# drprojects/DeepViewAgg

Hardware: AMD Instinct MI355X
Metric: points/sec fused fwd+bwd (1M pts, 32 views) (higher is better)
Workload: dtype bf16

## Files before the change

### deepviewagg_amd/_lib.py

```python
import ctypes
import os

_HERE = os.path.dirname(os.path.abspath(__file__))
LIB_PATH = os.environ.get("DVA_LIB_PATH") or os.path.join(_HERE, "csrc", "libdva_hip.so")

DVA_F32, DVA_BF16, DVA_F16 = 0, 1, 2
DVA_SUM, DVA_MEAN, DVA_MAX, DVA_MIN = 0, 1, 2, 3
REDUCE_CODE = {"sum": DVA_SUM, "add": DVA_SUM, "mean": DVA_MEAN, "max": DVA_MAX, "min": DVA_MIN}
CAMERA_CODE = {
    "s3dis_equirectangular": 0,
    "scannet": 1,
    "kitti360_perspective": 2,
    "kitti360_fisheye": 3,
}

_ERRORS = {
    -1: "DVA_ERR_INVALID (bad argument)",
    -2: "DVA_ERR_UNSUPPORTED",
    -3: "DVA_ERR_LAUNCH (HIP runtime error)",
    -4: "DVA_ERR_OVERFLOW (composite key does not fit int64)",
}


class DvaError(RuntimeError):
# ... 83 lines not shown
    "dva_rowbn_bwd_apply": (ctypes.c_int, [_vp, _vp, _vp, _vp, _vp, _vp, _i64, _i32, _f32, _i32, _vp]),
    "dva_bn_finalize": (ctypes.c_int, [_vp, ctypes.c_double, _vp, _vp, _vp, _vp, _vp, _f32, _f32, _i32, _i32, _vp,
                                       _vp]),
    "dva_scale_f64": (ctypes.c_int, [_vp, ctypes.c_double, _vp, _i32, _vp]),
    "dva_chain_prep": (ctypes.c_int, [_vp, _vp, _vp, _i32, _vp, _vp, _i32, _vp, _vp]),
    "dva_chain_tile_count": (ctypes.c_int, [_vp, _vp, _i32, _vp, _vp]),
    "dva_chain_tile_build": (ctypes.c_int, [_vp, _vp, _i32, _vp, _vp, _vp]),
    "dva_chain_moments": (ctypes.c_int, [_vp, _i64, _vp, _i32, _vp, _vp, _vp]),
    "dva_chain_stats2": (ctypes.c_int, [_vp, _vp, _vp, _vp, _vp, _vp, _vp, _vp, _vp, _vp, _i64, _vp]),
    "dva_chain_pooled": (ctypes.c_int, [_vp, _vp, _vp, _vp, _i64, _vp]),
    "dva_chain_stats": (ctypes.c_int, [_i32, _vp, _vp, _vp, _vp, _vp, _vp, _vp, _vp, _vp, _vp, _i64, _i64, _vp]),
    "dva_chain_stats_a2": (ctypes.c_int, [_i32, _vp, _vp, _vp, _vp, _vp, _vp, _vp, _vp, _vp, _vp, _i64, _i64, _vp, _vp]),
    "dva_chain_score_stats_a2": (ctypes.c_int, [_vp] * 12 + [_i32, _i64, _i64, _vp]),
    "dva_chain_bwd_layer6_a2": (ctypes.c_int, [_vp] * 13 + [_i32, _i64, _i64, _vp]),
    "dva_chain_attn_fwd": (ctypes.c_int, [_vp] * 18 + [_i64, _i64, _i64, _i32, _i32, _i32, _f32, _vp]),
    "dva_chain_attn_bwd": (ctypes.c_int, [_vp] * 14 + [_i64, _i64, _i64, _i32, _i32, _i32, _f32, _vp]),
    "dva_chain_attn_fwd_dt": (ctypes.c_int, [_vp] * 18 + [_i64, _i64, _i64, _i32, _i32, _i32, _f32, _i32, _vp]),
    "dva_chain_attn_bwd_dt": (ctypes.c_int, [_vp] * 14 + [_i64, _i64, _i64, _i32, _i32, _i32, _f32, _i32, _vp]),
    "dva_chain_attn_bwd_f32": (ctypes.c_int, [_vp] * 14 + [_i64, _i64, _i64, _i32, _i32, _i32, _f32, _vp]),
    "dva_gather_segment_max_fwd": (ctypes.c_int, [_vp] * 5 + [_i64, _i64, _i64, _i32, _i32, _vp]),
    "dva_gather_segment_max_bwd": (ctypes.c_int, [_vp] * 8 + [_i64, _i64, _i64, _i32, _i32, _vp]),
    "dva_chain_keys": (ctypes.c_int, [_vp] * 12 + [_i64, _i64, _vp]),
    "dva_chain_keys_compat": (ctypes.c_int, [_vp] * 14 + [_i32, _f32, _i64, _i64, _vp]),
    "dva_chain_attn_fwd_keys": (ctypes.c_int, [_vp] * 12 + [_f32] + [_vp] * 8 + [_i64, _i64, _i64, _i32, _i32, _i32, _f32, _vp]),
    "dva_qkv_dquery": (ctypes.c_int, [_vp, _i32, _vp, _vp, _vp, _i64, _i64, _i32, _f32, _vp]),
    "dva_chain_score_stats_keys": (ctypes.c_int, [_vp] * 15 + [_i32, _f32, _i64, _i64, _vp]),
    "dva_chain_bwd_layer6_keys": (ctypes.c_int, [_vp] * 16 + [_i32, _f32, _i64, _i64, _vp]),
    "dva_qkv_compat": (ctypes.c_int, [_vp] * 4 + [_i64, _i32, _f32, _vp]),
    "dva_qkv_compat_bwd": (ctypes.c_int, [_vp] * 7 + [_i64, _i64, _i32, _f32, _vp]),
    "dva_chain_attn_bwd_planrec": (ctypes.c_int, [_vp] * 15 + [_i64, _i64, _i64, _i32, _i32, _i32, _f32, _vp]),
    "dva_plan_inverse": (ctypes.c_int, [_vp, _vp, _i64, _vp]),
    "dva_plan_split_table_bytes": (ctypes.c_int64, [_i64, _i64]),
    "dva_plan_split_build": (ctypes.c_int, [_vp, _i64, _i64, _vp, _vp, _vp, _i64, _vp, _i64, _vp]),
    "dva_plan_split_sort_records": (ctypes.c_int, [_vp, _vp, _i64, _i64, _vp, _vp, _i64, _vp, _vp, _vp]),
    "dva_plan_split_sort_records32": (ctypes.c_int, [_vp, _vp, _i64, _i64, _vp, _i64, _vp, _vp]),
    "dva_plan_split_rows_grad": (ctypes.c_int, [_vp, _vp, _i64, _i64, _vp, _i64, _vp, _i32, _i32, _i32, _i32, _vp]),
    "dva_chain_score_stats": (ctypes.c_int, [_vp] * 14 + [_i32, _i64, _i64, _vp]),
    "dva_chain_bwd_layer": (ctypes.c_int, [_i32] + [_vp] * 22 + [_i32, _i64, _i64, _vp]),
    "dva_gather_bilinear_taps_anchor": (ctypes.c_int, [_vp, _vp, _i64, _i32, _i32, _i32, _vp, _vp, _vp, _vp]),
    "dva_bilinear_taps_cat": (ctypes.c_int, [_i32, _vp, _vp, _vp, _vp, _vp, _vp, _vp, _i64, _vp, _vp, _vp, _vp]),
    "dva_anchor_rows_sum": (ctypes.c_int, [_vp, _vp, _vp, _vp, _vp, _i64, _i64, _i32, _i32, _vp]),
    "dva_anchor_combine": (ctypes.c_int, [_vp, _vp, _i32, _i32, _i32, _i32, _vp]),
    "dva_anchor_fixup": (ctypes.c_int, [_vp, _vp, _vp, _vp, _vp, _i64, _i32, _i32, _i32, _i32, _i32, _vp]),
    "dva_anchor_rows_sum_bn": (ctypes.c_int, [_vp] * 10 + [_i64, _i64, _i32, _vp]),
    "dva_anchor_fixup_bn": (ctypes.c_int, [_vp] * 8 + [_i64, _i32, _i32, _i32, _i32, _vp]),
    "dva_emod_prep": (ctypes.c_int, [_vp, _i32, _vp, _vp]),
    "dva_emod_stats": (ctypes.c_int, [_i32] + [_vp] * 9 + [_i64, _i64, _i32, _vp]),
    "dva_emod_attn_fwd": (ctypes.c_int, [_vp] * 23 + [_i64, _i64, _i64, _i32, _i32, _i32, _f32, _vp]),
    "dva_emod_attn_bwd": (ctypes.c_int, [_vp] * 20 + [_i64, _i64, _i64, _i32, _i32, _i32, _f32, _vp]),
    "dva_emod_stats1_plan": (ctypes.c_int, [_vp] * 6 + [_i64, _i64, _i32, _vp]),
    "dva_emod_bwd": (ctypes.c_int, [_i32] + [_vp] * 16 + [_i64, _i64, _i64, _i32, _i32, _vp]),
    "dva_chain_score_l6_stats": (ctypes.c_int, [_vp] * 16 + [_i32, _i64, _i64, _vp]),
    "dva_chain_l6_consts": (ctypes.c_int, [_vp] * 7),
    "dva_chain_bwd_layer5_merged": (ctypes.c_int, [_vp] * 18 + [_i32, _i64, _i64, _vp]),
    "dva_chain_route_stats": (ctypes.c_int, [_vp, _vp, _vp, _vp, _vp, _vp, _i64, _vp]),
    "dva_copy_ceiling": (ctypes.c_int, [_vp, _vp, _i64, _vp]),
    "dva_zero_unseen_rows": (ctypes.c_int, [_vp, _vp, _i64, _i64, _vp]),
    "dva_chain_bn_consts": (ctypes.c_int, [_vp, ctypes.c_double, _vp, _vp, _vp, _vp, _vp, ctypes.c_float, ctypes.c_float,
                                           _i32, _vp, _i32, _i32, _vp, _vp, _vp]),
    "dva_concat_cast_fwd": (ctypes.c_int, [_vp, _vp, _vp, _i64, _i32, _i32, _i32, _vp]),
    "dva_concat_cast_bwd": (ctypes.c_int, [_vp, _vp, _vp, _i64, _i32, _i32, _i32, _vp]),
    "dva_mapping_row_index": (ctypes.c_int, [_vp, _vp, _vp, _i32, ctypes.c_double, _i64, _i64, _i32, _i32, _i32, _vp, _vp]),
    "dva_view_gather_rows_grad_rec16": (ctypes.c_int, [_vp, _vp, _vp, _vp, _vp, _i64, _i64, _i32, _i32, _i32, _vp]),
    "dva_view_gather_rows_grad_rec16_to": (ctypes.c_int, [_vp, _vp, _vp, _vp, _vp, _i32, _i64, _i64, _i32, _i32, _i32, _vp]),
    "dva_chain_tile_chunks": (ctypes.c_int, [_vp, _i64, _i64, _i32, _vp, _vp]),
    "dva_chain_tile_offsets": (ctypes.c_int, [_vp, _i32, _vp, _vp, _vp]),
# ... 122 lines not shown
```

### deepviewagg_amd/csrc/dva_common.h

```cpp
#pragma once
#include <hip/hip_runtime.h>
#include <stdint.h>

#include <cstdlib>

#include "../../include/dva.h"

#define DVA_WAVE 64

#define DVA_CHECK_LAUNCH()                           \
  do {                                               \
    hipError_t e__ = hipGetLastError();              \
    if (e__ != hipSuccess) return DVA_ERR_LAUNCH;    \
  } while (0)

namespace dva {

static inline int tune_int(const char* name, int dflt) {
  const char* v = getenv(name);
  return v && *v ? atoi(v) : dflt;
}

typedef uint16_t bf16_t;

// ... 57 lines not shown
};
template <>
struct Elt<bf16_t> {
  static __device__ __forceinline__ float ld(const bf16_t* p, int64_t i) { return bf2f(p[i]); }
  static __device__ __forceinline__ void st(bf16_t* p, int64_t i, float v) { p[i] = f2bf(v); }
};
template <>
struct Elt<f16_t> {
  static __device__ __forceinline__ float ld(const f16_t* p, int64_t i) { return (float)p[i]; }
  static __device__ __forceinline__ void st(f16_t* p, int64_t i, float v) { p[i] = (f16_t)v; }
};

__host__ __device__ __forceinline__ int group_of_channel(int c, int C, int G) {
  if (G <= 1) return 0;
  if (G >= C) return c;
  const int base = C / G, rem = C % G;
  const int split = rem * (base + 1);
  return c < split ? c / (base + 1) : rem + (c - split) / base;
}
__host__ __device__ __forceinline__ int group_begin(int g, int C, int G) {
  if (g >= G) return C;
  if (G <= 1) return 0;
  if (G >= C) return g;
  const int base = C / G, rem = C % G;
  return g < rem ? g * (base + 1) : rem * (base + 1) + (g - rem) * base;
}

struct __attribute__((aligned(8))) PackedIdx {
  int32_t img;
  int16_t x;
  int16_t y;
};

static inline int blocks_for(int64_t n, int threads) { return (int)((n + threads - 1) / threads); }

}
```

### deepviewagg_amd/csrc/gather.hip

```cpp
#include "dva_common.h"

namespace dva {

__device__ __forceinline__ float floordiv_f32(float a, float b) {
  const float mod = fmodf(a, b);
  float div = __fdiv_rn(__fsub_rn(a, mod), b);
  if (mod != 0.f && ((b < 0.f) != (mod < 0.f))) div = __fsub_rn(div, 1.f);
  if (div != 0.f) {
    float fl = floorf(div);
    if (__fsub_rn(div, fl) > 0.5f) fl = __fadd_rn(fl, 1.f);
    return fl;
  }
  return copysignf(0.f, __fdiv_rn(a, b));
}

template <typename PIX>
__global__ __launch_bounds__(256) void pack_index_kernel(const int64_t* __restrict__ images,
                                                          const int64_t* __restrict__ atom_ptr,
                                                          const PIX* __restrict__ pixels,
                                                          double ratio, int64_t n_views,
                                                          PackedIdx* __restrict__ out) {
  for (int64_t v = blockIdx.x * (int64_t)blockDim.x + threadIdx.x; v < n_views;
       v += (int64_t)gridDim.x * blockDim.x) {
    const int32_t img = (int32_t)images[v];
    for (int64_t a = atom_ptr[v]; a < atom_ptr[v + 1]; ++a) {
      PackedIdx pi;
      pi.img = img;
      if (ratio == 1.0) {
        pi.x = (int16_t)pixels[2 * a];
        pi.y = (int16_t)pixels[2 * a + 1];
      } else {
        const float rf = (float)ratio;
        pi.x = (int16_t)floordiv_f32((float)pixels[2 * a], rf);
        pi.y = (int16_t)floordiv_f32((float)pixels[2 * a + 1], rf);
      }
      out[a] = pi;
    }
  }
}

template <typename PIX>
__global__ __launch_bounds__(256) void mapping_row_index_kernel(const int64_t* __restrict__ images,
                                                                 const int64_t* __restrict__ atom_ptr,
                                                                 const PIX* __restrict__ pixels, double ratio,
                                                                 int64_t n_views, int H, int W,
                                                                 int32_t* __restrict__ row_idx) {
  for (int64_t v = blockIdx.x * (int64_t)blockDim.x + threadIdx.x; v < n_views;
       v += (int64_t)gridDim.x * blockDim.x) {
    const int32_t img = (int32_t)images[v];
    for (int64_t a = atom_ptr[v]; a < atom_ptr[v + 1]; ++a) {
      int32_t x, y;
      if (ratio == 1.0) {
        x = (int32_t)pixels[2 * a];
        y = (int32_t)pixels[2 * a + 1];
      } else {
        const float rf = (float)ratio;
        x = (int32_t)(int16_t)floordiv_f32((float)pixels[2 * a], rf);
        y = (int32_t)(int16_t)floordiv_f32((float)pixels[2 * a + 1], rf);
      }
      row_idx[a] = (img * H + y) * W + x;
    }
  }
}

__global__ __launch_bounds__(256) void row_index_kernel(const PackedIdx* __restrict__ idx,
                                                         int64_t n_atoms, int H, int W,
                                                         int32_t row_offset,
                                                         int32_t* __restrict__ row_idx,
                                                         int32_t* __restrict__ counts) {
  for (int64_t p = blockIdx.x * (int64_t)blockDim.x + threadIdx.x; p < n_atoms;
       p += (int64_t)gridDim.x * blockDim.x) {
    const PackedIdx pi = idx[p];
    const int32_t r = (pi.img * H + pi.y) * W + pi.x;
    row_idx[p] = r + row_offset;
    if (counts) atomicAdd(&counts[r], 1);
  }
}

template <typename UNIT>
__global__ __launch_bounds__(256) void gather_nearest_fwd_kernel(const UNIT* __restrict__ x,
                                                                  const PackedIdx* __restrict__ idx,
                                                                  UNIT* __restrict__ out,
                                                                  int64_t n_atoms, int H, int W,
                                                                  int units_per_row) {
  const int64_t total = n_atoms * (int64_t)units_per_row;
  for (int64_t t = blockIdx.x * (int64_t)blockDim.x + threadIdx.x; t < total;
       t += (int64_t)gridDim.x * blockDim.x) {
    const int64_t p = t / units_per_row;
    const int u = (int)(t - p * units_per_row);
    const PackedIdx pi = idx[p];
    const int64_t pix = ((int64_t)pi.img * H + pi.y) * W + pi.x;
    out[t] = x[pix * units_per_row + u];
  }
}
// ... 800 lines not shown
```

### deepviewagg_amd/csrc/plan_split.hip

```cpp
#include "dva_common.h"

namespace dva {
namespace ps {

constexpr int IPT = 8;
constexpr int BINS = 512;
constexpr int LO_BITS = 9;
constexpr int HEAD_INTS = 4096;

static inline int tile_size() {
  static const int t = tune_int("DVA_PLAN_TILE", 4096) == 8192 ? 8192 : 4096;
  return t;
}

struct Layout {
  int64_t nt, nb, ntb;
  size_t off_tot, off_bstart, off_tstart, off_order, off_a, off_b, off_desc, total;
};

static inline bool eligible(int64_t n_views, int64_t n_rows) {
  return n_views > 0 && n_views <= 0x7fffffffLL && n_rows > BINS && n_rows <= (int64_t)BINS * BINS;
}

static inline Layout layout(int64_t n, int64_t n_rows) {
  Layout L;
  const int TILE = tile_size();
  L.nt = (n + TILE - 1) / TILE;
  L.nb = (n_rows + BINS - 1) / BINS;
  L.ntb = L.nt + L.nb;
  L.off_tot = 0;
  L.off_bstart = 512 * 4;
  L.off_tstart = (512 + 520) * 4;
  L.off_order = 2048 * 4;
  L.off_a = HEAD_INTS * 4;
  L.off_b = L.off_a + (size_t)L.nt * BINS * 4;
  L.off_desc = L.off_b + (size_t)L.ntb * BINS * 4;
  L.total = L.off_desc + (size_t)L.ntb * 16;
  return L;
}

template <int NT>
// ... 28 lines not shown

template <int TILE>
__global__ __launch_bounds__(TILE / IPT) void hist_hi_kernel(const uint32_t* __restrict__ keys, int64_t n, int nb,
                                                             int64_t nt, int32_t* __restrict__ offA) {
  constexpr int THREADS = TILE / IPT;
  __shared__ int h[BINS];
  for (int i = threadIdx.x; i < BINS; i += THREADS) h[i] = 0;
  __syncthreads();
  const int64_t base = (int64_t)blockIdx.x * TILE;
#pragma unroll
  for (int k = 0; k < IPT; ++k) {
    const int64_t e = base + k * THREADS + threadIdx.x;
    if (e < n) atomicAdd(&h[hi_digit(keys[e], nb)], 1);
  }
  __syncthreads();
  for (int i = threadIdx.x; i < nb; i += THREADS) offA[(int64_t)i * nt + blockIdx.x] = h[i];
}

__global__ __launch_bounds__(256) void scan_tiles_kernel(int32_t* __restrict__ off, int64_t nt, int32_t* __restrict__ tot) {
  __shared__ int s_w[4];
  int32_t* row = off + (int64_t)blockIdx.x * nt;
  int carry = 0;
  for (int64_t t0 = 0; t0 < nt; t0 += 256) {
    const int64_t t = t0 + threadIdx.x;
    const int v = t < nt ? row[t] : 0;
    int all;
    const int ex = block_excl_scan<256>(v, s_w, &all);
    if (t < nt) row[t] = carry + ex;
    carry += all;
  }
  if (threadIdx.x == 0) tot[blockIdx.x] = carry;
}

__global__ __launch_bounds__(BINS) void bucket_starts_kernel(const int32_t* __restrict__ tot, int nb, int TILE,
                                                             int32_t* __restrict__ bucket_start,
                                                             int32_t* __restrict__ tile_start, int4* __restrict__ desc,
                                                             int32_t* __restrict__ order) {
  __shared__ int s_w[BINS / 64];
  __shared__ int s_tot[BINS];
  const int d = threadIdx.x;
  const int v = d < nb ? tot[d] : 0;
  s_tot[d] = d < nb ? v : -1;
  __syncthreads();
  if (d < nb) {
    int before = 0;
    for (int j = 0; j < nb; ++j) {
      const int t = s_tot[j];
      before += (t > v || (t == v && j < d)) ? 1 : 0;
    }
    order[before] = d;
  }
  int all;
  const int bs = block_excl_scan<BINS>(v, s_w, &all);
  bucket_start[d] = bs;
  if (d == BINS - 1) bucket_start[BINS] = all;
  int allt;
  const int nt_b = (v + TILE - 1) / TILE;
  const int ts = block_excl_scan<BINS>(nt_b, s_w, &allt);
  tile_start[d] = ts;
  if (d == BINS - 1) tile_start[BINS] = allt;
  for (int j = 0; j < nt_b; ++j) {
    const int left = v - j * TILE;
    desc[ts + j] = make_int4(d, bs + j * TILE, left < TILE ? left : TILE, 0);
  }
}

__device__ __forceinline__ void tile_b(const int4* __restrict__ desc, int tb, int& b, int64_t& start, int& count) {
  const int4 d = desc[tb];
  b = rfl_i(d.x);
  start = (int64_t)rfl_i(d.y);
  count = rfl_i(d.z);
}

template <int TILE>
__global__ __launch_bounds__(TILE / IPT) void hist_lo_kernel(const uint16_t* __restrict__ lows, int nb,
                                                             const int32_t* __restrict__ tile_start,
                                                             const int4* __restrict__ desc, int32_t* __restrict__ offB) {
  constexpr int THREADS = TILE / IPT;
  __shared__ int h[BINS];
  if ((int)blockIdx.x >= tile_start[nb]) return;
  int b, count;
  int64_t start;
  tile_b(desc, blockIdx.x, b, start, count);
  for (int i = threadIdx.x; i < BINS; i += THREADS) h[i] = 0;
  __syncthreads();
#pragma unroll
  for (int k = 0; k < IPT; ++k) {
    const int i = k * THREADS + threadIdx.x;
    if (i < count) atomicAdd(&h[lows[start + i]], 1);
  }
  __syncthreads();
  for (int i = threadIdx.x; i < BINS; i += THREADS) offB[(int64_t)blockIdx.x * BINS + i] = h[i];
}

__global__ __launch_bounds__(BINS) void scan_rows_kernel(int32_t* __restrict__ offB, const int32_t* __restrict__ bucket_start,
                                                         const int32_t* __restrict__ tile_start, int64_t n_rows,
                                                         int64_t n_views, int32_t* __restrict__ row_ptr,
// ... 361 lines not shown
          raw[u] = make_float4(0.f, 0.f, 0.f, 0.f);
          if (in) raw[u] = *reinterpret_cast<const float4*>(gout + p * C + cl * 4);
        }
#pragma unroll
        for (int u = 0; u < U; ++u) {
          acc[rr][0] = fmaf(raw[u].x, sc[u], acc[rr][0]);
          acc[rr][1] = fmaf(raw[u].y, sc[u], acc[rr][1]);
          acc[rr][2] = fmaf(raw[u].z, sc[u], acc[rr][2]);
          acc[rr][3] = fmaf(raw[u].w, sc[u], acc[rr][3]);
        }
      }
    }
  }
#pragma unroll
  for (int rr = 0; rr < RPT; ++rr) {
    const int64_t r = (int64_t)b * BINS + grp + GROUPS * rr;
    if (r < n_rows)
      *reinterpret_cast<float4*>(grows + r * C + cl * 4) = make_float4(acc[rr][0], acc[rr][1], acc[rr][2], acc[rr][3]);
  }
}

template <int C, typename T>
static void bucket_rows_grad(const uint4* rec, const T* gout, T* grows, int64_t n_rows, int G, int nb,
                             const int32_t* bstart, const int32_t* order, hipStream_t s) {
  static const int bt = tune_int("DVA_PLAN_BT", 8192);
  if (bt == 2048)
    hipLaunchKernelGGL((bucket_rows_grad_kernel<C, 2048, T>), dim3(nb), dim3(1024), 0, s, rec, gout, grows, n_rows, G, bstart, order);
  else if (bt == 4096)
    hipLaunchKernelGGL((bucket_rows_grad_kernel<C, 4096, T>), dim3(nb), dim3(1024), 0, s, rec, gout, grows, n_rows, G, bstart, order);
  else
    hipLaunchKernelGGL((bucket_rows_grad_kernel<C, 8192, T>), dim3(nb), dim3(1024), 0, s, rec, gout, grows, n_rows, G, bstart, order);
}

}
}

namespace dva {
namespace ps {
struct Tables {
  int32_t *tot, *bstart, *tstart, *order, *offA, *offB;
  int4* desc;
};
static inline Tables tables_of(void* tables, const Layout& L) {
  char* tb = (char*)tables;
  return {(int32_t*)(tb + L.off_tot), (int32_t*)(tb + L.off_bstart), (int32_t*)(tb + L.off_tstart),
          (int32_t*)(tb + L.off_order), (int32_t*)(tb + L.off_a), (int32_t*)(tb + L.off_b), (int4*)(tb + L.off_desc)};
}

static inline bool xcd_on() {
  static const int on = tune_int("DVA_PLAN_XCD", 1);
  return on != 0;
}
static inline unsigned scatter_grid(int64_t tiles) { return (unsigned)(xcd_on() ? (tiles + 7) / 8 * 8 : tiles); }

template <int TILE>
static void build(const uint32_t* keys, int64_t n, int64_t n_rows, int32_t* row_ptr, int32_t* counts, const Layout& L,
                  const Tables& T, void* scratch, hipStream_t s) {
  constexpr int THREADS = TILE / IPT;
  const int nb = (int)L.nb;
  hipLaunchKernelGGL(hist_hi_kernel<TILE>, dim3((unsigned)L.nt), dim3(THREADS), 0, s, keys, n, nb, L.nt, T.offA);
  hipLaunchKernelGGL(scan_tiles_kernel, dim3(nb), dim3(256), 0, s, T.offA, L.nt, T.tot);
  hipLaunchKernelGGL(bucket_starts_kernel, dim3(1), dim3(BINS), 0, s, T.tot, nb, TILE, T.bstart, T.tstart, T.desc, T.order);
  hipLaunchKernelGGL((scatter_kernel<MODE_LOWS, TILE>), dim3(scatter_grid(L.nt)), dim3(THREADS), 0, s, keys,
                     (const uint4*)nullptr, scratch, n, nb, n_rows, L.nt, T.bstart, T.tstart, T.desc, T.offA,
                     (const int32_t*)nullptr, (int)xcd_on());
  hipLaunchKernelGGL(hist_lo_kernel<TILE>, dim3((unsigned)L.ntb), dim3(THREADS), 0, s, (const uint16_t*)scratch, nb,
                     T.tstart, T.desc, T.offB);
  hipLaunchKernelGGL(scan_rows_kernel, dim3(nb), dim3(BINS), 0, s, T.offB, T.bstart, T.tstart, n_rows, n, row_ptr, counts);
}

template <int TILE>
static void sort_records(const uint32_t* keys, const uint4* rec, int64_t n, int64_t n_rows, const int32_t* row_ptr,
                         const Layout& L, const Tables& T, void* buf, void* out, hipStream_t s) {
  constexpr int THREADS = TILE / IPT;
  const int nb = (int)L.nb;
  hipLaunchKernelGGL((scatter_kernel<MODE_REC_A, TILE>), dim3(scatter_grid(L.nt)), dim3(THREADS), 0, s, keys, rec,
                     buf, n, nb, n_rows, L.nt, T.bstart, T.tstart, T.desc, T.offA, (const int32_t*)nullptr,
                     (int)xcd_on());
  if (!out) return;
  hipLaunchKernelGGL((scatter_kernel<MODE_REC_B, TILE>), dim3(scatter_grid(L.ntb)), dim3(THREADS), 0, s,
                     (const uint32_t*)nullptr, (const uint4*)buf, out, n, nb, n_rows, L.nt, T.bstart, T.tstart, T.desc,
                     T.offB, row_ptr, (int)xcd_on());
}
}
}

using namespace dva;

extern "C" {

int64_t dva_plan_split_table_bytes(int64_t n_views, int64_t n_rows) {
  if (n_views < 0 || n_rows < 0) return DVA_ERR_INVALID;
  if (!ps::eligible(n_views, n_rows)) return DVA_ERR_UNSUPPORTED;
  return (int64_t)ps::layout(n_views, n_rows).total;
}

int dva_plan_split_build(const int32_t* row_idx, int64_t n_views, int64_t n_rows, int32_t* row_ptr, int32_t* counts,
                         void* tables, int64_t tables_bytes, void* scratch, int64_t scratch_bytes, void* stream) {
  if (n_views < 0 || n_rows < 0) return DVA_ERR_INVALID;
  if (!ps::eligible(n_views, n_rows)) return DVA_ERR_UNSUPPORTED;
  if (!row_idx || !row_ptr || !tables || !scratch) return DVA_ERR_INVALID;
  const ps::Layout L = ps::layout(n_views, n_rows);
  if ((int64_t)L.total > tables_bytes || scratch_bytes < n_views * 2) return DVA_ERR_INVALID;
  const ps::Tables T = ps::tables_of(tables, L);
  if (ps::tile_size() == 4096)
    ps::build<4096>((const uint32_t*)row_idx, n_views, n_rows, row_ptr, counts, L, T, scratch, (hipStream_t)stream);
  else
    ps::build<8192>((const uint32_t*)row_idx, n_views, n_rows, row_ptr, counts, L, T, scratch, (hipStream_t)stream);
  DVA_CHECK_LAUNCH();
  return DVA_OK;
}

int dva_plan_split_sort_records(const int32_t* row_idx, const void* rec, int64_t n_views, int64_t n_rows,
                                const int32_t* row_ptr, const void* tables, int64_t tables_bytes, void* buf,
                                void* rec_sorted, void* stream) {
  if (n_views < 0 || n_rows < 0) return DVA_ERR_INVALID;
  if (!ps::eligible(n_views, n_rows)) return DVA_ERR_UNSUPPORTED;
  if (!rec || !row_ptr || !tables || !buf || buf == rec || buf == rec_sorted) return DVA_ERR_INVALID;
  if (((uintptr_t)rec % 16) || ((uintptr_t)buf % 16) || ((uintptr_t)rec_sorted % 16)) return DVA_ERR_UNSUPPORTED;
  const ps::Layout L = ps::layout(n_views, n_rows);
  if ((int64_t)L.total > tables_bytes) return DVA_ERR_INVALID;
  const ps::Tables T = ps::tables_of(const_cast<void*>(tables), L);
  if (ps::tile_size() == 4096)
    ps::sort_records<4096>((const uint32_t*)row_idx, (const uint4*)rec, n_views, n_rows, row_ptr, L, T, buf, rec_sorted,
                           (hipStream_t)stream);
  else
    ps::sort_records<8192>((const uint32_t*)row_idx, (const uint4*)rec, n_views, n_rows, row_ptr, L, T, buf, rec_sorted,
                           (hipStream_t)stream);
  DVA_CHECK_LAUNCH();
  return DVA_OK;
}

int dva_plan_split_sort_records32(const int32_t* row_idx, const void* rec, int64_t n_views, int64_t n_rows,
                                  const void* tables, int64_t tables_bytes, void* buf, void* stream) {
  if (n_views < 0 || n_rows < 0) return DVA_ERR_INVALID;
  if (!ps::eligible(n_views, n_rows) || ps::tile_size() != 4096) return DVA_ERR_UNSUPPORTED;
  if (!row_idx || !rec || !tables || !buf || buf == rec) return DVA_ERR_INVALID;
  if (((uintptr_t)rec % 16) || ((uintptr_t)buf % 16)) return DVA_ERR_UNSUPPORTED;
  const ps::Layout L = ps::layout(n_views, n_rows);
  if ((int64_t)L.total > tables_bytes) return DVA_ERR_INVALID;
  const ps::Tables T = ps::tables_of(const_cast<void*>(tables), L);
// ... 52 lines not shown
```

### deepviewagg_amd/csrc/segment.hip

```cpp
#include "dva_common.h"

namespace dva {

template <typename T, int REDUCE>
__global__ __launch_bounds__(256) void segment_csr_fwd_kernel(const T* __restrict__ src,
                                                               const int64_t* __restrict__ ptr,
                                                               T* __restrict__ out,
                                                               int32_t* __restrict__ arg,
                                                               int64_t n_groups, int C) {
  const int64_t total = n_groups * (int64_t)C;
  for (int64_t t = blockIdx.x * (int64_t)blockDim.x + threadIdx.x; t < total;
       t += (int64_t)gridDim.x * blockDim.x) {
    const int64_t g = t / C;
    const int c = (int)(t - g * C);
    const int64_t beg = ptr[g], end = ptr[g + 1];
    float acc;
    int64_t best = -1;
    if (REDUCE == DVA_SUM || REDUCE == DVA_MEAN) {
      acc = 0.f;
      for (int64_t r = beg; r < end; ++r) acc += Elt<T>::ld(src, r * C + c);
      if (REDUCE == DVA_MEAN && end > beg) acc /= (float)(end - beg);
    } else {
      acc = 0.f;
      for (int64_t r = beg; r < end; ++r) {
// ... 250 lines not shown
}

template <typename T>
static int launch_segment_bwd(const void* gout, const int64_t* ptr, const int32_t* arg, void* gsrc,
                              int64_t n, int C, int reduce, hipStream_t s) {
  const bool vec = vec_ok<T>(gout, gsrc, C);
  const int grid = grid_for(n * (int64_t)(vec ? C / SVec<T>::N : C));
#define DVA_L(R)                                                                                         \
  do {                                                                                                   \
    if (vec)                                                                                             \
      hipLaunchKernelGGL((segment_csr_bwd_vec_kernel<T, R>), dim3(grid), dim3(256), 0, s, (const T*)gout, \
                         ptr, arg, (T*)gsrc, n, C);                                                      \
    else                                                                                                 \
      hipLaunchKernelGGL((segment_csr_bwd_kernel<T, R>), dim3(grid), dim3(256), 0, s, (const T*)gout,    \
                         ptr, arg, (T*)gsrc, n, C);                                                      \
  } while (0)
  switch (reduce) {
    case DVA_SUM: DVA_L(DVA_SUM); break;
    case DVA_MEAN: DVA_L(DVA_MEAN); break;
    case DVA_MAX: DVA_L(DVA_MAX); break;
    case DVA_MIN: DVA_L(DVA_MIN); break;
    default: return DVA_ERR_INVALID;
  }
#undef DVA_L
  return DVA_OK;
}

}

using namespace dva;

extern "C" {

int dva_version(void) { return 307; }

int dva_device_count(void) {
  int n = 0;
  hipError_t e = hipGetDeviceCount(&n);
  if (e == hipErrorNoDevice) return 0;
  if (e != hipSuccess) return DVA_ERR_LAUNCH;
  return n;
}

int dva_segment_csr_fwd(const void* src, const int64_t* ptr, void* out, int32_t* arg,
                        int64_t n_groups, int32_t C, int32_t dtype, int32_t reduce, void* stream) {
  if (n_groups < 0 || C < 0 || !ptr) return DVA_ERR_INVALID;
  if (reduce < DVA_SUM || reduce > DVA_MIN) return DVA_ERR_INVALID;
  if (n_groups == 0 || C == 0) return DVA_OK;
  if (!out) return DVA_ERR_INVALID;
  int rc;
  if (dtype == DVA_F32)
    rc = launch_segment_fwd<float>(src, ptr, out, arg, n_groups, C, reduce, (hipStream_t)stream);
  else if (dtype == DVA_BF16)
    rc = launch_segment_fwd<bf16_t>(src, ptr, out, arg, n_groups, C, reduce, (hipStream_t)stream);
  else if (dtype == DVA_F16)
    rc = launch_segment_fwd<f16_t>(src, ptr, out, arg, n_groups, C, reduce, (hipStream_t)stream);
  else
    return DVA_ERR_INVALID;
  if (rc) return rc;
  DVA_CHECK_LAUNCH();
  return DVA_OK;
}

int dva_segment_csr_bwd(const void* grad_out, const int64_t* ptr, const int32_t* arg,
                        void* grad_src, int64_t n_groups, int32_t C, int32_t dtype,
                        int32_t reduce, void* stream) {
  if (n_groups < 0 || C < 0 || !ptr) return DVA_ERR_INVALID;
// ... 71 lines not shown
```

### deepviewagg_amd/ops.py

```python
import os

import threading

import torch

from . import _lib
from ._lib import check, dtype_code, ptr, require_device, stream_of

ROWS_GRAD_ALGO = 0
ATTENTION_ALGO = 0


class KernelTimer:

    def __init__(self, only=None):
        self.records = []
        self.only = None if only is None else set(only)

    def launch(self, name, nbytes):
        if self.only is not None and name not in self.only:
            return _NO_TIMER
        return _TimedLaunch(self, name, nbytes)

    def summary(self):
# ... 642 lines not shown
    with _timed("view_gather_rows_grad", V * ((4 if perm is not None else 0) + 16 + C * 2) + R * (C * 2 + 4)):
        check(lib.dva_view_gather_rows_grad_rec16_to(ptr(gout), ptr(perm), ptr(row_ptr), ptr(rec), ptr(g), dtype_code(g),
                                                     R, V, C, G, dtype_code(gout), stream),
              "dva_view_gather_rows_grad_rec16_to")
    return g


def csr_expand(csr_idx, n_views):
    lib = _lib.load()
    require_device(csr_idx)
    vp = torch.empty(n_views, dtype=torch.int32, device=csr_idx.device)
    check(lib.dva_csr_expand(ptr(csr_idx), csr_idx.shape[0] - 1, ptr(vp), stream_of(csr_idx)),
          "dva_csr_expand")
    return vp


def gather_row_index(packed_idx, B, H, W, row_offset=0, with_counts=True, with_plan=False, split=True):
    lib = _lib.load()
    require_device(packed_idx)
    P = packed_idx.shape[0]
    row_idx = torch.empty(P, dtype=torch.int32, device=packed_idx.device)
    hist = with_counts and not with_plan
    counts = torch.zeros(B * H * W, dtype=torch.int32, device=packed_idx.device) if hist else None
    with _timed("gather_row_index", P * 12):
        check(lib.dva_gather_row_index(ptr(packed_idx), P, B, H, W, int(row_offset), ptr(row_idx),
                                       ptr(counts), stream_of(packed_idx)), "dva_gather_row_index")
    if with_plan:
        assert row_offset == 0, "a plan is built over the rows of one map"
        plan, counts = row_plan(row_idx, B * H * W, with_counts, split)
        return row_idx, counts, plan
    return row_idx, counts


def mapping_row_index(images, atom_ptr, pixels, ratio, B, H, W, with_counts=True, with_plan=True, split=True):
    lib = _lib.load()
    require_device(images, atom_ptr, pixels)
    images = images.contiguous()
    atom_ptr = _check_ptr(atom_ptr)
    pixels = pixels.contiguous()
    if pixels.dtype not in (torch.int16, torch.int32, torch.int64):
        raise TypeError(f"pixels must be int16/int32/int64, got {pixels.dtype}")
    V, P = images.shape[0], pixels.shape[0]
    row_idx = torch.empty(P, dtype=torch.int32, device=pixels.device)
    with _timed("gather_row_index", V * 28 + P * 8):
        check(lib.dva_mapping_row_index(ptr(images), ptr(atom_ptr), ptr(pixels), pixels.element_size(), float(ratio),
                                        V, P, B, H, W, ptr(row_idx), stream_of(pixels)), "dva_mapping_row_index")
    if not with_plan:
        return row_idx, None, None
    plan, counts = row_plan(row_idx, B * H * W, with_counts, split)
    return row_idx, counts, plan


class GatheredFeatures:

    def __init__(self, rows, row_idx, counts, exact, plan=None):
        self.rows, self.row_idx, self.counts, self.exact = rows, row_idx, counts, exact
        self.plan = plan

    def with_rows(self, rows):
        assert rows.shape[0] == self.rows.shape[0]
        plan = self.plan
        if isinstance(plan, SplitPlan) and not split_plan_serves(rows.dtype, rows.shape[1]):
            plan = None
        return GatheredFeatures(rows, self.row_idx, self.counts, self.exact, plan)

    @property
    def shape(self):
        return torch.Size((self.row_idx.shape[0], self.rows.shape[1]))

    @property
    def device(self):
        return self.rows.device

    @property
    def dtype(self):
        return self.rows.dtype

    def dim(self):
        return 2

    def materialize(self):
        return gather_rows(self.rows, self.row_idx)

    @staticmethod
    def cat(items, order=None):
        offs, rows, idx, cnt = 0, [], [], []
        for it in items:
            rows.append(it.rows)
            idx.append(it.row_idx + offs)
            cnt.append(it.counts)
            offs += it.rows.shape[0]
        if len(items) == 1 and order is None:
            return items[0]
        row_idx = torch.cat(idx)
        if order is not None:
            row_idx = row_idx[order]
        return GatheredFeatures(torch.cat(rows, dim=0), row_idx.contiguous(), torch.cat(cnt),
                                all(it.exact for it in items))


def lazy_gather_nearest(x, packed_idx, exact):
    assert x.dim() == 4
    B, C, H, W = x.shape
    rows = x.permute(0, 2, 3, 1).reshape(B * H * W, C)
    row_idx, counts, plan = gather_row_index(packed_idx, B, H, W, with_plan=True,
                                             split=bool(exact) and split_plan_serves(x.dtype, C))
    return GatheredFeatures(rows, row_idx, counts, exact, plan)


def lazy_gather_nearest_mapping(x, images, atom_ptr, pixels, ratio, exact):
    assert x.dim() == 4
    B, C, H, W = x.shape
    rows = x.permute(0, 2, 3, 1).reshape(B * H * W, C)
    row_idx, counts, plan = mapping_row_index(images, atom_ptr, pixels, ratio, B, H, W,
                                              split=bool(exact) and split_plan_serves(x.dtype, C))
    return GatheredFeatures(rows, row_idx, counts, exact, plan)


class _GatherSegmentMax(torch.autograd.Function):

    @staticmethod
    def forward(ctx, rows, row_idx, atom_ptr, plan):
        lib = _lib.load()
        require_device(rows, row_idx, atom_ptr)
        rows = rows.contiguous()
        (R, C), V, P = rows.shape, atom_ptr.shape[0] - 1, row_idx.shape[0]
        out = torch.empty((V, C), dtype=rows.dtype, device=rows.device)
        arg = torch.empty((V, C), dtype=torch.int16, device=rows.device)
        es = rows.element_size()
        with _timed("gather_segment_max_fwd", P * (4 + C * es) + V * (8 + C * (es + 2))):
            check(lib.dva_gather_segment_max_fwd(ptr(rows), ptr(row_idx), ptr(atom_ptr), ptr(out), ptr(arg), V, P, R, C,
                                                 dtype_code(rows), stream_of(rows)), "dva_gather_segment_max_fwd")
        ctx.save_for_backward(row_idx, atom_ptr, arg)
        ctx.meta = (R, C, rows.dtype)
        ctx.plan = plan
        return out

    @staticmethod
    def backward(ctx, gout):
        lib = _lib.load()
        row_idx, atom_ptr, arg = ctx.saved_tensors
        R, C, dt = ctx.meta
        gout = gout.contiguous().to(dt)
        V, P = atom_ptr.shape[0] - 1, row_idx.shape[0]
        es = gout.element_size()
        groups = C // (16 // es)
        if SEGMENT_MAX_ATOMICS or groups & (groups - 1) or groups > 64 or P > 0x7fffffff:
            grows = torch.zeros((R, C), dtype=torch.float32, device=gout.device)
# ... 610 lines not shown
```

### include/dva.h

```cpp
#ifndef DVA_H_
#define DVA_H_

#include <stdint.h>

#ifdef __cplusplus
extern "C" {
#endif

#define DVA_OK 0
#define DVA_ERR_INVALID (-1)
#define DVA_ERR_UNSUPPORTED (-2)
#define DVA_ERR_LAUNCH (-3)
#define DVA_ERR_OVERFLOW (-4)

#define DVA_F32 0
#define DVA_BF16 1
#define DVA_F16 2

#define DVA_SUM 0
#define DVA_MEAN 1
#define DVA_MAX 2
#define DVA_MIN 3

#define DVA_CAM_EQUIRECT 0
// ... 56 lines not shown
                           float* gate, int32_t* amax, int64_t n_points, int64_t n_views, int32_t C,
                           int32_t G, int32_t scaling, float eps, int32_t dtype, int32_t algo,
                           void* stream);

int dva_view_attention_bwd(const void* grad_out, const void* val, const float* compat,
                           const float* att, const float* gate, const int32_t* amax,
                           const int64_t* ptr, const float* gate_w, const float* gate_b,
                           void* grad_val, float* grad_compat, float* grad_gate_wb,
                           int64_t n_points, int64_t n_views, int32_t C, int32_t G, int32_t scaling,
                           int32_t dtype, int32_t algo, void* stream);

int dva_view_gather_attention_fwd(const void* rows, const int32_t* row_idx, const float* compat,
                                  const int64_t* ptr, const float* gate_w, const float* gate_b,
                                  void* out, float* att, float* gate, int32_t* amax,
                                  int64_t n_points, int64_t n_views, int32_t C, int32_t G,
                                  int32_t scaling, float eps, int32_t dtype, int32_t algo,
                                  void* stream);
int dva_view_gather_attention_bwd(const void* grad_out, const void* rows, const int32_t* row_idx,
                                  const float* compat, const float* att, const float* gate,
                                  const int32_t* amax, const int64_t* ptr, const float* gate_w,
                                  const float* gate_b, float* grad_rows, float* grad_compat,
                                  float* grad_gate_wb, float* view_rec, int32_t rec_stride,
                                  int64_t n_points, int64_t n_views, int32_t C, int32_t G,
                                  int32_t scaling, int32_t dtype, int32_t algo, void* stream);

int64_t dva_row_plan_workspace_bytes(int64_t n_views, int64_t n_rows);
int dva_row_plan(const int32_t* row_idx, int64_t n_views, int64_t n_rows, int32_t* perm,
                 int32_t* row_ptr, int32_t* counts, void* workspace, int64_t workspace_bytes,
                 void* stream);

int64_t dva_plan_split_table_bytes(int64_t n_views, int64_t n_rows);
int dva_plan_split_build(const int32_t* row_idx, int64_t n_views, int64_t n_rows, int32_t* row_ptr, int32_t* counts,
                         void* tables, int64_t tables_bytes, void* scratch, int64_t scratch_bytes, void* stream);
int dva_plan_split_sort_records(const int32_t* row_idx, const void* rec, int64_t n_views, int64_t n_rows,
                                const int32_t* row_ptr, const void* tables, int64_t tables_bytes, void* buf,
                                void* rec_sorted, void* stream);
int dva_plan_split_sort_records32(const int32_t* row_idx, const void* rec, int64_t n_views, int64_t n_rows,
                                  const void* tables, int64_t tables_bytes, void* buf, void* stream);
int dva_plan_split_rows_grad(const void* grad_out, const void* bucket_rec, int64_t n_views, int64_t n_rows,
                             const void* tables, int64_t tables_bytes, void* grad_rows, int32_t C, int32_t G, int32_t dtype,
                             int32_t out_dtype, void* stream);

int dva_view_gather_rows_grad(const void* grad_out, const float* att, const float* gate,
                              const int32_t* view_point, const int32_t* perm, const int32_t* row_ptr,
                              const float* view_rec, int32_t rec_stride, float* grad_rows,
                              int64_t n_rows, int64_t n_views, int32_t C, int32_t G, int32_t dtype,
                              void* stream);

int dva_view_gather_rows_grad_rec16(const void* grad_out, const int32_t* perm, const int32_t* row_ptr,
                                    const void* view_rec16, float* grad_rows, int64_t n_rows, int64_t n_views,
                                    int32_t C, int32_t G, int32_t dtype, void* stream);
int dva_view_gather_rows_grad_rec16_to(const void* grad_out, const int32_t* perm, const int32_t* row_ptr,
                                       const void* view_rec16, void* grad_rows, int32_t out_dtype, int64_t n_rows,
                                       int64_t n_views, int32_t C, int32_t G, int32_t dtype, void* stream);

int dva_gather_rows_sum(const void* grad_out, const int32_t* perm, const int32_t* row_ptr,
                        const float* weights, int32_t atom_shift, float* grad_rows, int64_t n_rows,
                        int64_t n_atoms, int32_t C, int32_t dtype, void* stream);
int dva_gather_bilinear_taps_anchor(const void* packed_idx, const float* coords, int64_t n_atoms, int32_t B,
                                    int32_t H, int32_t W, int32_t* rows, float* weights, int32_t* anchors,
                                    void* stream);
int dva_bilinear_taps_cat(int32_t n_settings, const void* const* tap_rows, const void* const* tap_weights,
                          const void* const* anchors, const int64_t* n_views, const int64_t* n_rows,
                          const int64_t* n_anchors, const int64_t* order, int64_t n_views_total, int32_t* rows_out,
                          float* weights_out, int32_t* anchors_out, void* stream);
int dva_anchor_rows_sum(const void* grad_out, const int32_t* perm, const int32_t* row_ptr, const float* weights,
// ... 337 lines not shown
```

Measured before the change: 101.5 million.

## Fuse mapping row-index computation into split-plan histogram build

Adds a fused path that computes row indices from images and pixels and builds the first-pass histogram in the same kernel. The per-bucket scan and the bucket-start ordering are merged into one launch using a last-block ticket. A dedicated low-digit histogram kernel fills in row_ptr and counts. The aim is to cut kernel launches and extra passes over row_idx when building the mapping plan. It applies only when exact is set and there is one pixel per view, and it depends on a hand-written cross-block atomic and fence protocol.

```diff
diff --git a/deepviewagg_amd/_lib.py b/deepviewagg_amd/_lib.py
--- a/deepviewagg_amd/_lib.py
+++ b/deepviewagg_amd/_lib.py
@@ -139,6 +139,8 @@
     "dva_plan_inverse": (ctypes.c_int, [_vp, _vp, _i64, _vp]),
     "dva_plan_split_table_bytes": (ctypes.c_int64, [_i64, _i64]),
     "dva_plan_split_build": (ctypes.c_int, [_vp, _i64, _i64, _vp, _vp, _vp, _i64, _vp, _i64, _vp]),
+    "dva_mapping_split_build": (ctypes.c_int, [_vp, _vp, _i32, ctypes.c_double, _i64, _i32, _i32, _i32, _vp, _vp, _vp, _vp,
+                                               _i64, _vp, _i64, _vp]),
     "dva_plan_split_sort_records": (ctypes.c_int, [_vp, _vp, _i64, _i64, _vp, _vp, _i64, _vp, _vp, _vp]),
     "dva_plan_split_sort_records32": (ctypes.c_int, [_vp, _vp, _i64, _i64, _vp, _i64, _vp, _vp]),
     "dva_plan_split_rows_grad": (ctypes.c_int, [_vp, _vp, _i64, _i64, _vp, _i64, _vp, _i32, _i32, _i32, _i32, _vp]),
diff --git a/deepviewagg_amd/csrc/dva_common.h b/deepviewagg_amd/csrc/dva_common.h
--- a/deepviewagg_amd/csrc/dva_common.h
+++ b/deepviewagg_amd/csrc/dva_common.h
@@ -113,6 +113,32 @@
   int16_t y;
 };
 
+__device__ __forceinline__ float floordiv_f32(float a, float b) {
+  const float mod = fmodf(a, b);
+  float div = __fdiv_rn(__fsub_rn(a, mod), b);
+  if (mod != 0.f && ((b < 0.f) != (mod < 0.f))) div = __fsub_rn(div, 1.f);
+  if (div != 0.f) {
+    float fl = floorf(div);
+    if (__fsub_rn(div, fl) > 0.5f) fl = __fadd_rn(fl, 1.f);
+    return fl;
+  }
+  return copysignf(0.f, __fdiv_rn(a, b));
+}
+
+template <typename PIX>
+__device__ __forceinline__ int32_t mapped_row(int32_t img, PIX px, PIX py, double ratio, int H, int W) {
+  int32_t x, y;
+  if (ratio == 1.0) {
+    x = (int32_t)px;
+    y = (int32_t)py;
+  } else {
+    const float rf = (float)ratio;
+    x = (int32_t)(int16_t)floordiv_f32((float)px, rf);
+    y = (int32_t)(int16_t)floordiv_f32((float)py, rf);
+  }
+  return (img * H + y) * W + x;
+}
+
 static inline int blocks_for(int64_t n, int threads) { return (int)((n + threads - 1) / threads); }
 
 }
diff --git a/deepviewagg_amd/csrc/gather.hip b/deepviewagg_amd/csrc/gather.hip
--- a/deepviewagg_amd/csrc/gather.hip
+++ b/deepviewagg_amd/csrc/gather.hip
@@ -1,18 +1,6 @@
 #include "dva_common.h"
 
 namespace dva {
-
-__device__ __forceinline__ float floordiv_f32(float a, float b) {
-  const float mod = fmodf(a, b);
-  float div = __fdiv_rn(__fsub_rn(a, mod), b);
-  if (mod != 0.f && ((b < 0.f) != (mod < 0.f))) div = __fsub_rn(div, 1.f);
-  if (div != 0.f) {
-    float fl = floorf(div);
-    if (__fsub_rn(div, fl) > 0.5f) fl = __fadd_rn(fl, 1.f);
-    return fl;
-  }
-  return copysignf(0.f, __fdiv_rn(a, b));
-}
 
 template <typename PIX>
 __global__ __launch_bounds__(256) void pack_index_kernel(const int64_t* __restrict__ images,
@@ -48,18 +36,8 @@
   for (int64_t v = blockIdx.x * (int64_t)blockDim.x + threadIdx.x; v < n_views;
        v += (int64_t)gridDim.x * blockDim.x) {
     const int32_t img = (int32_t)images[v];
-    for (int64_t a = atom_ptr[v]; a < atom_ptr[v + 1]; ++a) {
-      int32_t x, y;
-      if (ratio == 1.0) {
-        x = (int32_t)pixels[2 * a];
-        y = (int32_t)pixels[2 * a + 1];
-      } else {
-        const float rf = (float)ratio;
-        x = (int32_t)(int16_t)floordiv_f32((float)pixels[2 * a], rf);
-        y = (int32_t)(int16_t)floordiv_f32((float)pixels[2 * a + 1], rf);
-      }
-      row_idx[a] = (img * H + y) * W + x;
-    }
+    for (int64_t a = atom_ptr[v]; a < atom_ptr[v + 1]; ++a)
+      row_idx[a] = mapped_row(img, pixels[2 * a], pixels[2 * a + 1], ratio, H, W);
   }
 }
 
diff --git a/deepviewagg_amd/csrc/plan_split.hip b/deepviewagg_amd/csrc/plan_split.hip
--- a/deepviewagg_amd/csrc/plan_split.hip
+++ b/deepviewagg_amd/csrc/plan_split.hip
@@ -7,6 +7,7 @@
 constexpr int BINS = 512;
 constexpr int LO_BITS = 9;
 constexpr int HEAD_INTS = 4096;
+constexpr int TICKET_INT = HEAD_INTS - 1;
 
 static inline int tile_size() {
   static const int t = tune_int("DVA_PLAN_TILE", 4096) == 8192 ? 8192 : 4096;
@@ -101,21 +102,25 @@
   if (threadIdx.x == 0) tot[blockIdx.x] = carry;
 }
 
-__global__ __launch_bounds__(BINS) void bucket_starts_kernel(const int32_t* __restrict__ tot, int nb, int TILE,
-                                                             int32_t* __restrict__ bucket_start,
-                                                             int32_t* __restrict__ tile_start, int4* __restrict__ desc,
-                                                             int32_t* __restrict__ order) {
-  __shared__ int s_w[BINS / 64];
-  __shared__ int s_tot[BINS];
+__device__ __forceinline__ void bucket_starts_body(const int32_t* __restrict__ tot, int nb, int TILE,
+                                                   int32_t* __restrict__ bucket_start, int32_t* __restrict__ tile_start,
+                                                   int4* __restrict__ desc, int32_t* __restrict__ order, int* s_w,
+                                                   int* s_tot) {
   const int d = threadIdx.x;
   const int v = d < nb ? tot[d] : 0;
   s_tot[d] = d < nb ? v : -1;
   __syncthreads();
   if (d < nb) {
+    const int4* s4 = reinterpret_cast<const int4*>(s_tot);
     int before = 0;
-    for (int j = 0; j < nb; ++j) {
-      const int t = s_tot[j];
-      before += (t > v || (t == v && j < d)) ? 1 : 0;
+#pragma unroll 8
+    for (int j4 = 0; j4 < BINS / 4; ++j4) {
+      const int4 t = s4[j4];
+      const int j = 4 * j4;
+      before += (t.x > v || (t.x == v && j < d)) ? 1 : 0;
+      before += (t.y > v || (t.y == v && j + 1 < d)) ? 1 : 0;
+      before += (t.z > v || (t.z == v && j + 2 < d)) ? 1 : 0;
+      before += (t.w > v || (t.w == v && j + 3 < d)) ? 1 : 0;
     }
     order[before] = d;
   }
@@ -132,6 +137,15 @@
     const int left = v - j * TILE;
     desc[ts + j] = make_int4(d, bs + j * TILE, left < TILE ? left : TILE, 0);
   }
+}
+
+__global__ __launch_bounds__(BINS) void bucket_starts_kernel(const int32_t* __restrict__ tot, int nb, int TILE,
+                                                             int32_t* __restrict__ bucket_start,
+                                                             int32_t* __restrict__ tile_start, int4* __restrict__ desc,
+                                                             int32_t* __restrict__ order) {
+  __shared__ int s_w[BINS / 64];
+  __shared__ __attribute__((aligned(16))) int s_tot[BINS];
+  bucket_starts_body(tot, nb, TILE, bucket_start, tile_start, desc, order, s_w, s_tot);
 }
 
 __device__ __forceinline__ void tile_b(const int4* __restrict__ desc, int tb, int& b, int64_t& start, int& count) {
@@ -559,6 +573,154 @@
     hipLaunchKernelGGL((bucket_rows_grad_kernel<C, 8192, T>), dim3(nb), dim3(1024), 0, s, rec, gout, grows, n_rows, G, bstart, order);
 }
 
+template <typename PIX, int TILE>
+__global__ __launch_bounds__(TILE / IPT) void map_hist_kernel(const int64_t* __restrict__ images, const PIX* __restrict__ pixels,
+                                                              double ratio, int64_t n, int H, int W, int nb, int64_t nt,
+                                                              int32_t* __restrict__ row_idx, int32_t* __restrict__ offA,
+                                                              int32_t* __restrict__ ticket) {
+  constexpr int THREADS = TILE / IPT;
+  __shared__ int h[BINS];
+  const int tid = threadIdx.x;
+  const int64_t base = (int64_t)blockIdx.x * TILE;
+  int64_t img[IPT];
+  PIX px[IPT], py[IPT];
+#pragma unroll
+  for (int k = 0; k < IPT; ++k) {
+    const int64_t e = base + k * THREADS + tid;
+    const int64_t g = e < n ? e : n - 1;
+    img[k] = images[g];
+    px[k] = pixels[2 * g];
+    py[k] = pixels[2 * g + 1];
+  }
+  for (int i = tid; i < BINS; i += THREADS) h[i] = 0;
+  if (blockIdx.x == 0 && tid == 0) *ticket = 0;
+  __syncthreads();
+#pragma unroll
+  for (int k = 0; k < IPT; ++k) {
+    const int64_t e = base + k * THREADS + tid;
+    if (e < n) {
+      const int32_t r = mapped_row((int32_t)img[k], px[k], py[k], ratio, H, W);
+      row_idx[e] = r;
+      atomicAdd(&h[hi_digit((uint32_t)r, nb)], 1);
+    }
+  }
+  __syncthreads();
+  for (int i = tid; i < nb; i += THREADS) offA[(int64_t)i * nt + blockIdx.x] = h[i];
+}
+
+__global__ __launch_bounds__(BINS) void scan_starts_kernel(int32_t* __restrict__ off, int64_t nt, int nb, int TILE,
+                                                           int32_t* __restrict__ tot, int32_t* __restrict__ bucket_start,
+                                                           int32_t* __restrict__ tile_start, int4* __restrict__ desc,
+                                                           int32_t* __restrict__ order, int32_t* __restrict__ ticket) {
+  constexpr int K = 16, CH = BINS * K;
+  __shared__ __attribute__((aligned(16))) int s[CH + CH / 32];
+  __shared__ int s_w[BINS / 64];
+  __shared__ int s_last;
+  const int tid = threadIdx.x;
+  int32_t* row = off + (int64_t)blockIdx.x * nt;
+  int carry = 0;
+  for (int64_t c0 = 0; c0 < nt; c0 += CH) {
+#pragma unroll
+    for (int k = 0; k < K; ++k) {
+      const int i = k * BINS + tid;
+      const int64_t g = c0 + i;
+      s[i + (i >> 5)] = g < nt ? row[g] : 0;
+    }
+    __syncthreads();
+    int v[K], sum = 0;
+#pragma unroll
+    for (int j = 0; j < K; ++j) {
+      const int i = tid * K + j;
+      v[j] = s[i + (i >> 5)];
+      sum += v[j];
+    }
+    int all;
+    int run = carry + block_excl_scan<BINS>(sum, s_w, &all);
+#pragma unroll
+    for (int j = 0; j < K; ++j) {
+      const int i = tid * K + j;
+      s[i + (i >> 5)] = run;
+      run += v[j];
+    }
+    __syncthreads();
+#pragma unroll
+    for (int k = 0; k < K; ++k) {
+      const int i = k * BINS + tid;
+      const int64_t g = c0 + i;
+      if (g < nt) row[g] = s[i + (i >> 5)];
+    }
+    carry += all;
+    __syncthreads();
+  }
+  if (tid == 0) tot[blockIdx.x] = carry;
+  asm volatile("s_waitcnt vmcnt(0)" ::: "memory");
+  __syncthreads();
+  if (tid == 0) {
+    __builtin_amdgcn_fence(__ATOMIC_RELEASE, "agent");
+    asm volatile("s_waitcnt vmcnt(0)" ::: "memory");
+    const int t = __hip_atomic_fetch_add(ticket, 1, __ATOMIC_RELAXED, __HIP_MEMORY_SCOPE_AGENT);
+    s_last = t == nb - 1;
+    if (t == nb - 1) {
+      __builtin_amdgcn_fence(__ATOMIC_ACQUIRE, "agent");
+      asm volatile("s_waitcnt vmcnt(0)" ::: "memory");
+    }
+  }
+  __syncthreads();
+  if (!s_last) return;
+  bucket_starts_body(tot, nb, TILE, bucket_start, tile_start, desc, order, s_w, s);
+}
+
+template <int TILE>
+__global__ __launch_bounds__(1024) void bucket_lo_kernel(const uint16_t* __restrict__ lows,
+                                                         const int32_t* __restrict__ bucket_start,
+                                                         const int32_t* __restrict__ tile_start, int64_t n_rows,
+                                                         int64_t n_views, int32_t* __restrict__ offB,
+                                                         int32_t* __restrict__ row_ptr, int32_t* __restrict__ counts) {
+  constexpr int THREADS = 1024, CH = 65536, K = CH / TILE, PER = CH / THREADS, U = 16;
+  __shared__ int h[K][BINS];
+  __shared__ int s_w[THREADS / 64];
+  const int b = blockIdx.x, tid = threadIdx.x;
+  const int tb0 = tile_start[b], tb1 = tile_start[b + 1];
+  const int64_t b0 = bucket_start[b];
+  const int ne = bucket_start[b + 1] - bucket_start[b];
+  int run = 0;
+  for (int c0 = 0; c0 < ne; c0 += CH) {
+#pragma unroll
+    for (int k = 0; k < K * BINS / THREADS; ++k) (&h[0][0])[k * THREADS + tid] = 0;
+    __syncthreads();
+    for (int k0 = 0; k0 < PER; k0 += U) {
+      uint16_t dg[U];
+#pragma unroll
+      for (int u = 0; u < U; ++u) {
+        const int i = c0 + (k0 + u) * THREADS + tid;
+        dg[u] = lows[b0 + (i < ne ? i : 0)];
+      }
+#pragma unroll
+      for (int u = 0; u < U; ++u) {
+        const int j = (k0 + u) * THREADS + tid;
+        if (c0 + j < ne) atomicAdd(&h[j / TILE][dg[u] & (BINS - 1)], 1);
+      }
+    }
+    __syncthreads();
+    if (tid < BINS) {
+#pragma unroll
+      for (int j = 0; j < K; ++j) {
+        const int tb = tb0 + c0 / TILE + j;
+        if (tb < tb1) {
+          offB[(int64_t)tb * BINS + tid] = run;
+          run += h[j][tid];
+        }
+      }
+    }
+    __syncthreads();
+  }
+  const int64_t r = (int64_t)b * BINS + tid;
+  if (tid < BINS && counts && r < n_rows) counts[r] = run;
+  const int excl = block_excl_scan<THREADS>(tid < BINS ? run : 0, s_w);
+  if (tid < BINS && r <= n_rows) row_ptr[r] = bucket_start[b] + excl;
+  if (r + 1 == n_rows && tid == BINS - 1) row_ptr[n_rows] = (int32_t)n_views;
+}
+
 }
 }
 
@@ -596,6 +758,44 @@
   hipLaunchKernelGGL(scan_rows_kernel, dim3(nb), dim3(BINS), 0, s, T.offB, T.bstart, T.tstart, n_rows, n, row_ptr, counts);
 }
 
+template <int TILE, typename PIX>
+static void mapping_build(const int64_t* images, const PIX* pixels, double ratio, int64_t n, int H, int W, int64_t n_rows,
+                          int32_t* row_idx, int32_t* row_ptr, int32_t* counts, const Layout& L, const Tables& T,
+                          int32_t* ticket, void* lows, hipStream_t s) {
+  constexpr int THREADS = TILE / IPT;
+  const int nb = (int)L.nb;
+  hipLaunchKernelGGL((map_hist_kernel<PIX, TILE>), dim3((unsigned)L.nt), dim3(THREADS), 0, s, images, pixels, ratio, n, H,
+                     W, nb, L.nt, row_idx, T.offA, ticket);
+  hipLaunchKernelGGL(scan_starts_kernel, dim3(nb), dim3(BINS), 0, s, T.offA, L.nt, nb, TILE, T.tot, T.bstart, T.tstart,
+                     T.desc, T.order, ticket);
+  hipLaunchKernelGGL((scatter_kernel<MODE_LOWS, TILE>), dim3(scatter_grid(L.nt)), dim3(THREADS), 0, s,
+                     (const uint32_t*)row_idx, (const uint4*)nullptr, lows, n, nb, n_rows, L.nt, T.bstart, T.tstart,
+                     T.desc, T.offA, (const int32_t*)nullptr, (int)xcd_on());
+  hipLaunchKernelGGL(bucket_lo_kernel<TILE>, dim3(nb), dim3(1024), 0, s, (const uint16_t*)lows, T.bstart, T.tstart,
+                     n_rows, n, T.offB, row_ptr, counts);
+}
+
+template <int TILE>
+static int mapping_build_px(const int64_t* images, const void* pixels, int32_t pix_bytes, double ratio, int64_t n, int H,
+                            int W, int64_t n_rows, int32_t* row_idx, int32_t* row_ptr, int32_t* counts, const Layout& L,
+                            const Tables& T, int32_t* ticket, void* lows, hipStream_t s) {
+  switch (pix_bytes) {
+    case 2:
+      mapping_build<TILE>(images, (const int16_t*)pixels, ratio, n, H, W, n_rows, row_idx, row_ptr, counts, L, T, ticket,
+                          lows, s);
+      return DVA_OK;
+    case 4:
+      mapping_build<TILE>(images, (const int32_t*)pixels, ratio, n, H, W, n_rows, row_idx, row_ptr, counts, L, T, ticket,
+                          lows, s);
+      return DVA_OK;
+    case 8:
+      mapping_build<TILE>(images, (const int64_t*)pixels, ratio, n, H, W, n_rows, row_idx, row_ptr, counts, L, T, ticket,
+                          lows, s);
+      return DVA_OK;
+  }
+  return DVA_ERR_INVALID;
+}
+
 template <int TILE>
 static void sort_records(const uint32_t* keys, const uint4* rec, int64_t n, int64_t n_rows, const int32_t* row_ptr,
                          const Layout& L, const Tables& T, void* buf, void* out, hipStream_t s) {
@@ -634,6 +834,30 @@
     ps::build<4096>((const uint32_t*)row_idx, n_views, n_rows, row_ptr, counts, L, T, scratch, (hipStream_t)stream);
   else
     ps::build<8192>((const uint32_t*)row_idx, n_views, n_rows, row_ptr, counts, L, T, scratch, (hipStream_t)stream);
+  DVA_CHECK_LAUNCH();
+  return DVA_OK;
+}
+
+int dva_mapping_split_build(const int64_t* images, const void* pixels, int32_t pix_bytes, double ratio, int64_t n_views,
+                            int32_t B, int32_t H, int32_t W, int32_t* row_idx, int32_t* row_ptr, int32_t* counts,
+                            void* tables, int64_t tables_bytes, void* lows, int64_t lows_bytes, void* stream) {
+  if (n_views < 0 || !(ratio >= 1.0) || B < 0 || H < 0 || W < 0) return DVA_ERR_INVALID;
+  if (pix_bytes != 2 && pix_bytes != 4 && pix_bytes != 8) return DVA_ERR_INVALID;
+  if ((int64_t)B * H * W > 0x7fffffffLL || H > 32767 || W > 32767) return DVA_ERR_UNSUPPORTED;
+  const int64_t n_rows = (int64_t)B * H * W;
+  if (!ps::eligible(n_views, n_rows)) return DVA_ERR_UNSUPPORTED;
+  if (!images || !pixels || !row_idx || !row_ptr || !tables || !lows) return DVA_ERR_INVALID;
+  const ps::Layout L = ps::layout(n_views, n_rows);
+  if ((int64_t)L.total > tables_bytes || lows_bytes < n_views * 2) return DVA_ERR_INVALID;
+  const ps::Tables T = ps::tables_of(tables, L);
+  int32_t* ticket = (int32_t*)tables + ps::TICKET_INT;
+  hipStream_t s = (hipStream_t)stream;
+  const int rc = ps::tile_size() == 4096
+                     ? ps::mapping_build_px<4096>(images, pixels, pix_bytes, ratio, n_views, H, W, n_rows, row_idx, row_ptr,
+                                                  counts, L, T, ticket, lows, s)
+                     : ps::mapping_build_px<8192>(images, pixels, pix_bytes, ratio, n_views, H, W, n_rows, row_idx, row_ptr,
+                                                  counts, L, T, ticket, lows, s);
+  if (rc != DVA_OK) return rc;
   DVA_CHECK_LAUNCH();
   return DVA_OK;
 }
diff --git a/deepviewagg_amd/csrc/segment.hip b/deepviewagg_amd/csrc/segment.hip
--- a/deepviewagg_amd/csrc/segment.hip
+++ b/deepviewagg_amd/csrc/segment.hip
@@ -306,7 +306,7 @@
 
 extern "C" {
 
-int dva_version(void) { return 307; }
+int dva_version(void) { return 308; }
 
 int dva_device_count(void) {
   int n = 0;
diff --git a/deepviewagg_amd/ops.py b/deepviewagg_amd/ops.py
--- a/deepviewagg_amd/ops.py
+++ b/deepviewagg_amd/ops.py
@@ -698,7 +698,8 @@
     return row_idx, counts
 
 
-def mapping_row_index(images, atom_ptr, pixels, ratio, B, H, W, with_counts=True, with_plan=True, split=True):
+def mapping_row_index(images, atom_ptr, pixels, ratio, B, H, W, with_counts=True, with_plan=True, split=True,
+                      exact=False):
     lib = _lib.load()
     require_device(images, atom_ptr, pixels)
     images = images.contiguous()
@@ -708,12 +709,26 @@
         raise TypeError(f"pixels must be int16/int32/int64, got {pixels.dtype}")
     V, P = images.shape[0], pixels.shape[0]
     row_idx = torch.empty(P, dtype=torch.int32, device=pixels.device)
+    n_rows = B * H * W
+    if with_plan and split and exact and P == V and SPLIT_PLAN and _split_plan_pays(V, n_rows):
+        nbytes = int(lib.dva_plan_split_table_bytes(V, n_rows))
+        if nbytes > 0:
+            dev = pixels.device
+            row_ptr = torch.empty(n_rows + 1, dtype=torch.int32, device=dev)
+            counts = torch.empty(n_rows, dtype=torch.int32, device=dev) if with_counts else None
+            tables = torch.empty(nbytes, dtype=torch.uint8, device=dev)
+            lows = torch.empty(V, dtype=torch.int16, device=dev)
+            with _timed("mapping_split_build", V * 26):
+                check(lib.dva_mapping_split_build(ptr(images), ptr(pixels), pixels.element_size(), float(ratio), V, B, H,
+                                                  W, ptr(row_idx), ptr(row_ptr), ptr(counts), ptr(tables), nbytes,
+                                                  ptr(lows), V * 2, stream_of(pixels)), "dva_mapping_split_build")
+            return row_idx, counts, SplitPlan(row_idx, n_rows, row_ptr, tables)
     with _timed("gather_row_index", V * 28 + P * 8):
         check(lib.dva_mapping_row_index(ptr(images), ptr(atom_ptr), ptr(pixels), pixels.element_size(), float(ratio),
                                         V, P, B, H, W, ptr(row_idx), stream_of(pixels)), "dva_mapping_row_index")
     if not with_plan:
         return row_idx, None, None
-    plan, counts = row_plan(row_idx, B * H * W, with_counts, split)
+    plan, counts = row_plan(row_idx, n_rows, with_counts, split)
     return row_idx, counts, plan
 
 
@@ -779,7 +794,7 @@
     B, C, H, W = x.shape
     rows = x.permute(0, 2, 3, 1).reshape(B * H * W, C)
     row_idx, counts, plan = mapping_row_index(images, atom_ptr, pixels, ratio, B, H, W,
-                                              split=bool(exact) and split_plan_serves(x.dtype, C))
+                                              split=bool(exact) and split_plan_serves(x.dtype, C), exact=bool(exact))
     return GatheredFeatures(rows, row_idx, counts, exact, plan)
 
 
diff --git a/include/dva.h b/include/dva.h
--- a/include/dva.h
+++ b/include/dva.h
@@ -112,6 +112,9 @@
 int64_t dva_plan_split_table_bytes(int64_t n_views, int64_t n_rows);
 int dva_plan_split_build(const int32_t* row_idx, int64_t n_views, int64_t n_rows, int32_t* row_ptr, int32_t* counts,
                          void* tables, int64_t tables_bytes, void* scratch, int64_t scratch_bytes, void* stream);
+int dva_mapping_split_build(const int64_t* images, const void* pixels, int32_t pix_bytes, double ratio, int64_t n_views,
+                            int32_t B, int32_t H, int32_t W, int32_t* row_idx, int32_t* row_ptr, int32_t* counts,
+                            void* tables, int64_t tables_bytes, void* lows, int64_t lows_bytes, void* stream);
 int dva_plan_split_sort_records(const int32_t* row_idx, const void* rec, int64_t n_views, int64_t n_rows,
                                 const int32_t* row_ptr, const void* tables, int64_t tables_bytes, void* buf,
                                 void* rec_sorted, void* stream);
```

Result: faster. 102.6 million, median of 6 (+1.1%).
